# clownrat6/Tissue-Image-Segmentation

Hardware: NVIDIA B200
Metric: postproc+eval tiles/s @1000x1000 (DIST MoNuSeg config) (higher is better)
Workload: dtype u8/int32 labels, fp32 softmax, fp64 IoU

## Files before the change

tissue-image-segmentation_b200/csrc/watershed.cu:

```cuda
#include "watershed.cuh"

namespace tiseg {

#define FULL 0xffffffffu

__global__ void k_blob_init(BlobInfo b, int W) {
    int n = blockIdx.y;
    long long o = (long long)n * b.KS;
    int k = b.count[n];
    for (int i = blockIdx.x * blockDim.x + threadIdx.x; i <= k; i += gridDim.x * blockDim.x) {
        b.root[o + i] = 0; b.ymax[o + i] = -1; b.xmin[o + i] = W; b.xmax[o + i] = -1; b.area[o + i] = 0;
        if (b.lmin) { b.lmin[o + i] = 0x7fffffff; b.lmax[o + i] = 0; }
    }
}

__global__ void __launch_bounds__(TISEG_THREADS)
k_blob_roots(Geom g, const unsigned* __restrict__ bits, const int* __restrict__ rank, BlobInfo b) {
    const long long words = (long long)g.H * g.SEG;
    const long long t = (long long)blockIdx.x * blockDim.x + threadIdx.x;
    if (t >= words) return;
    const int n = blockIdx.y;
    unsigned m = bits[(long long)n * words + t];
    if (!m) return;
    const int y = (int)(t / g.SEG), seg = (int)(t - (long long)y * g.SEG);
// ... 32 lines not shown
    __syncthreads();
    for (int base = 1; base <= k; base += 256) {
        int i = base + threadIdx.x;
        int v = i <= k ? b.area[o + i] : 0;
        s[threadIdx.x] = v;
        __syncthreads();
        for (int d = 1; d < 256; d <<= 1) {
            int t = threadIdx.x >= d ? s[threadIdx.x - d] : 0;
            __syncthreads();
            s[threadIdx.x] += t;
            __syncthreads();
        }
        int incl = s[threadIdx.x];
        int c0 = carry;
        if (i <= k) b.off[o + i] = c0 + incl - v;
        __syncthreads();
        if (threadIdx.x == 255) carry = c0 + incl;
        __syncthreads();
    }
}

__global__ void __launch_bounds__(TISEG_THREADS)
k_blob_runs(Geom g, BitPlanes p, const int* __restrict__ par, const int* __restrict__ rank, BlobInfo b, int32_t* __restrict__ out) {
    const long long words = (long long)g.H * g.SEG;
    const long long t = (long long)blockIdx.x * blockDim.x + threadIdx.x;
    if (t >= words) return;
    const int n = blockIdx.y;
    const unsigned F = p.F[(long long)n * words + t];
    if (!F) return;
    const int y = (int)(t / g.SEG), seg = (int)(t - (long long)y * g.SEG);
    for (unsigned m = F & ~(F << 1); m; m &= m - 1) {
        const int a = __ffs(m) - 1;
        const unsigned rest = ~F >> a;
        const int len = rest ? __ffs(rest) - 1 : 32 - a;
        const int x = seg * 32 + a;
        const long long o = (long long)n * b.KS + blob_id_at(p, g, n, par, rank, y, x);
        const int lo = b.lmin[o], hi = b.lmax[o];
        if (lo < hi) {
            atomicMax(&b.ymax[o], y);
            atomicMin(&b.xmin[o], x);
            atomicMax(&b.xmax[o], x + len - 1);
            atomicAdd(&b.area[o], len);
        } else {
            const int lab = lo == hi ? lo : 0;
            int32_t* dst = out + (long long)n * g.P + (long long)y * g.W + x;
            for (int k = 0; k < len; ++k) dst[k] = lab;
        }
    }
}
__global__ void __launch_bounds__(TISEG_THREADS)
k_ws_seed(long long total, const int32_t* __restrict__ markers, const int* __restrict__ par, int32_t* __restrict__ out, bool vec) {
    const long long i = flat4_index();
    if (i >= total) return;
    Pack4<int> m = ld4(markers, i, total, vec), p = ld4(par, i, total, vec), o;
#pragma unroll
    for (int k = 0; k < 4; ++k) o.v[k] = p.v[k] >= 0 ? m.v[k] : 0;
    st4(out, i, total, vec, o);
}

#define WS_NOTIN 0xFFFFu
#define WS_UNLAB 0xFFFEu
#define WS_END 0xFFFFu

#define WS_MAXCLS 16
extern __shared__ __align__(16) unsigned char ws_smem[];

struct FloodWork {
    long long* items;
    long long* gen;
    long long* ovf;
    int* count;
    int* offset;
    int* fill;
    int* cursor;
    int* ngen;
    int* gcursor;
};
#define WK_INTS (4 * WS_MAXCLS + 4)

__device__ __forceinline__ long long blob_cells(const BlobInfo& b, long long ko, int bid, int W) {
    int h = b.ymax[ko + bid] - b.root[ko + bid] / W + 1, w = b.xmax[ko + bid] - b.xmin[ko + bid] + 1;
    return (long long)(w + 2) * (h + 2);
}
__device__ __forceinline__ int blob_class(long long cells, int arena, int slots) {
    if (cells > arena) return -1;
    int cls = arena / (int)cells - 1;
    return cls >= slots ? slots - 1 : cls;
}

__global__ void __launch_bounds__(TISEG_THREADS)
k_huge_clean(Geom g, BitPlanes p, const int* __restrict__ par, const int* __restrict__ rank, BlobInfo b,
             const unsigned* __restrict__ seed_bits, long long gen_cap, int32_t* __restrict__ out) {
    const long long words = (long long)g.H * g.SEG;
    const long long t = (long long)blockIdx.x * blockDim.x + threadIdx.x;
    if (t >= words) return;
    const int y = (int)(t / g.SEG), seg = (int)(t - (long long)y * g.SEG);
    FOR_TILES(true, g, n) {
        const unsigned F = p.F[(long long)n * words + t];
        const unsigned seeds = seed_bits[(long long)n * words + t];
        for (unsigned m = F & ~(F << 1); m; m &= m - 1) {
            const int a = __ffs(m) - 1;
            const unsigned rest = ~F >> a;
            const int len = rest ? __ffs(rest) - 1 : 32 - a;
            const int x = seg * 32 + a;
            const long long ko = (long long)n * b.KS;
            const int bid = blob_id_at(p, g, n, par, rank, y, x);
            if (b.lmin[ko + bid] >= b.lmax[ko + bid] || blob_cells(b, ko, bid, g.W) <= gen_cap) continue;
            int32_t* dst = out + (long long)n * g.P + (long long)y * g.W + x;
            for (int k = 0; k < len; ++k) if (!((seeds >> (a + k)) & 1u)) dst[k] = 0;
        }
    }
}

__global__ void k_flood_count(BlobInfo b, int W, FloodWork wk, int arena, int slots) {
    int n = blockIdx.y;
    long long ko = (long long)n * b.KS;
    int B = b.count[n];
    for (int bid = 1 + blockIdx.x * blockDim.x + threadIdx.x; bid <= B; bid += gridDim.x * blockDim.x) {
        if (b.lmin && b.lmin[ko + bid] >= b.lmax[ko + bid]) {
            if (b.first && b.lmax[ko + bid] > 0 && b.lmin[ko + bid] == b.lmax[ko + bid])
                atomicMin(&b.first[ko + b.lmax[ko + bid]], b.root[ko + bid]);
            continue;
        }
        int cls = blob_class(blob_cells(b, ko, bid, W), arena, slots);
        if (cls >= 0) atomicAdd(&wk.count[cls], 1);
    }
}
__global__ void k_flood_offsets(FloodWork wk) {
    if (threadIdx.x == 0) {
        int acc = 0;
        for (int k = 0; k < WS_MAXCLS; ++k) { wk.offset[k] = acc; acc += wk.count[k]; }
    }
}
__global__ void k_flood_scatter(BlobInfo b, int W, FloodWork wk, int arena, int slots, long long gen_cap, int* huge) {
    int n = blockIdx.y;
    long long ko = (long long)n * b.KS;
    int B = b.count[n];
    for (int bid = 1 + blockIdx.x * blockDim.x + threadIdx.x; bid <= B; bid += gridDim.x * blockDim.x) {
        if (b.lmin && b.lmin[ko + bid] >= b.lmax[ko + bid]) continue;
        const long long cells = blob_cells(b, ko, bid, W);
        int cls = blob_class(cells, arena, slots);
        long long item = ((long long)n << 32) | (unsigned)bid;
        if (cls >= 0) wk.items[wk.offset[cls] + atomicAdd(&wk.fill[cls], 1)] = item;
        else {
            wk.gen[atomicAdd(wk.ngen, 1)] = item;
            if (huge && cells > gen_cap && atomicExch(&huge[n], 1) == 0) huge[gridDim.y + atomicAdd(&huge[2 * gridDim.y], 1)] = n;
        }
    }
}
__global__ void __launch_bounds__(TISEG_THREADS)
k_label_clean(Geom g, const unsigned* __restrict__ keep, int32_t* __restrict__ lab) {
    const long long words = (long long)g.H * g.SEG;
    const long long wi = (long long)blockIdx.x * TISEG_WARPS_PER_BLOCK + (threadIdx.x >> 5);
    const int lane = threadIdx.x & 31;
    if (wi >= words) return;
    const int y = (int)(wi / g.SEG), seg = (int)(wi - (long long)y * g.SEG), x = seg * 32 + lane;
    FOR_TILES(true, g, n) {
        const unsigned w = keep[(long long)n * words + wi];
        if (x < g.W && !((w >> lane) & 1u)) lab[(long long)n * g.P + (long long)y * g.W + x] = 0;
    }
}
int label_clean_listed(tiseg_ctx* c, const Geom& g, const int* list, const int* count, const unsigned* keep, int32_t* lab) {
    Geom gl = listed_geom(g, list, count);
    TISEG_LAUNCH(c, k_label_clean, dim3((unsigned)(((long long)g.H * g.SEG + TISEG_WARPS_PER_BLOCK - 1) / TISEG_WARPS_PER_BLOCK), 1),
                 TISEG_THREADS, 0, gl, keep, lab);
    return TISEG_OK;
}

__device__ __forceinline__ int fdiv(int j, unsigned magic) { return (int)__umulhi((unsigned)j, magic); }

struct SeedStats { int lmn, lmx, jseed; };
struct InForest {
    static constexpr bool kMasked = false;
    const int* tp; int root;
    __device__ __forceinline__ int load(int gi) const { return tp[gi]; }
    __device__ __forceinline__ bool in(int v) const { return v == root; }
    __device__ __forceinline__ bool seed(int, unsigned, int, int ov) const { return ov != 0; }
    __device__ __forceinline__ unsigned seed_word(int, int) const { return 0u; }
};
struct InMask {
    static constexpr bool kMasked = true;
    const uint8_t* m; const int* seed_blob; const unsigned* sbits; int SEG; int bid;
    __device__ __forceinline__ int load(int gi) const { return m[gi]; }
    __device__ __forceinline__ bool in(int v) const { return v < 255; }
    __device__ __forceinline__ unsigned seed_word(int y, int x) const { return sbits[y * SEG + (x >> 5)]; }
    __device__ __forceinline__ bool seed(int gi, unsigned word, int x, int) const {
        return ((word >> (x & 31)) & 1u) && seed_blob[gi] == bid;
    }
};

template <class IT, class LT>
__device__ __forceinline__ SeedStats stage_copy(int tid, int nthr, int W, const IT* __restrict__ I, const InForest mb,
                                                const int32_t* __restrict__ o, int root,
                                                int y0, int x0, int w, int h, unsigned short* lab, LT* lvl) {
    SeedStats st; st.lmn = 0x7fffffff; st.lmx = 0; st.jseed = 0x7fffffff;
    const int wp = w + 2, cells = wp * (h + 2);
    const unsigned magic = 0xFFFFFFFFu / (unsigned)wp + 1u;
    for (int j0 = 0; j0 < cells; j0 += 8 * nthr) {
        int gi[8];
        bool in[8];
#pragma unroll
        for (int u = 0; u < 8; ++u) {
            const int j = j0 + u * nthr + tid;
            const int ly = fdiv(j, magic), lx = j - ly * wp;
            in[u] = j < cells && ly >= 1 && ly <= h && lx >= 1 && lx <= w;
            gi[u] = in[u] ? (y0 + ly - 1) * W + x0 + lx - 1 : root;
        }
        int tpv[8], ov[8];
        IT iv[8];
#pragma unroll
        for (int u = 0; u < 8; ++u) { tpv[u] = mb.load(gi[u]); iv[u] = I[gi[u]]; ov[u] = o[gi[u]]; }
#pragma unroll
        for (int u = 0; u < 8; ++u) {
            const int j = j0 + u * nthr + tid;
            if (j < cells) {
                const bool inblob = in[u] && mb.in(tpv[u]);
                const bool seed = inblob && mb.seed(gi[u], 0u, 0, ov[u]);
                lab[j] = (unsigned short)(inblob ? (seed ? (unsigned)j : WS_UNLAB) : WS_NOTIN);
                lvl[j] = (LT)iv[u];
                if (seed) { st.lmn = min(st.lmn, ov[u]); st.lmx = max(st.lmx, ov[u]); st.jseed = min(st.jseed, j); }
            }
        }
    }
    return st;
}

__device__ __forceinline__ bool fill_if_single_marker(int lane, SeedStats st, int cells, unsigned short* lab) {
#pragma unroll
    for (int d = 16; d; d >>= 1) {
// ... 118 lines not shown
        for (int u = 0; u < 8; ++u) if (dst[u] >= 0) o[dst[u]] = val[u];
    }
}

template <class MB>
__device__ __forceinline__ void flood_blob_global(int lane, int W, int H, const uint8_t* __restrict__ I,
                                                  const MB mb, int32_t* o, int* nx, int root, int y0,
                                                  int y1, int x0, int x1, int* head, int* tail, int* first = nullptr) {
    for (int i = lane; i < 256; i += 32) { head[i] = -1; tail[i] = -1; }
    __syncwarp();
    int cur = 256;
    for (int y = y0; y <= y1; ++y) {
        for (int xb = x0; xb <= x1; xb += 32) {
            int x = xb + lane;
            bool seed = false;
            int lv = 0;
            if (x <= x1) {
                int idx = y * W + x;
                if (mb.in(mb.load(idx)) && mb.seed(idx, MB::kMasked ? mb.seed_word(y, x) : 0u, x, o[idx])) { seed = true; lv = I[idx]; }
            }
            unsigned m = __ballot_sync(FULL, seed);
            while (m) {
                int src = __ffs(m) - 1;
                m &= m - 1;
                int slv = __shfl_sync(FULL, lv, src);
                if (lane == 0) {
                    int pix = y * W + xb + src;
                    if (first) atomicMin(&first[o[pix]], pix);
                    nx[pix] = -1;
                    int t = tail[slv];
                    if (t < 0) head[slv] = pix; else nx[t] = pix;
                    tail[slv] = pix;
                    if (slv < cur) cur = slv;
                }
            }
        }
    }
    if (lane == 0) {
        for (;;) {
            while (cur < 256 && head[cur] < 0) ++cur;
            if (cur >= 256) break;
            const int pix = head[cur];
            const int nxt = nx[pix];
            head[cur] = nxt;
            if (nxt < 0) tail[cur] = -1;
            const int lab_g = o[pix];
            const int y = pix / W, x = pix - y * W;
            const int nb[4] = {pix - W, pix - 1, pix + 1, pix + W};
            const bool ok[4] = {y > 0, x > 0, x + 1 < W, y + 1 < H};
            int ov[4], lv[4];
            bool pin[4];
#pragma unroll
            for (int k = 0; k < 4; ++k) {
                pin[k] = false; ov[k] = 1; lv[k] = 0;
                if (ok[k]) { pin[k] = mb.in(mb.load(nb[k])); ov[k] = o[nb[k]]; lv[k] = I[nb[k]]; }
            }
#pragma unroll
            for (int k = 0; k < 4; ++k) {
                if (pin[k] && ov[k] == 0) {
                    o[nb[k]] = lab_g;
                    if (first) atomicMin(&first[lab_g], nb[k]);
                    nx[nb[k]] = -1;
                    int t = tail[lv[k]];
                    if (t < 0) head[lv[k]] = nb[k]; else nx[t] = nb[k];
                    tail[lv[k]] = nb[k];
                    if (lv[k] < cur) cur = lv[k];
                }
            }
        }
    }
    __syncwarp();
}

#define WP_WARPS 16
#define WP_BIG_WARPS 4
#define WP_ARENA 4224
#define WP_SMALL_ARENA (WP_ARENA / 3)
#define WP_SMALL_CLS 2
#define WP_META_BYTES (256 * 2 * 2 + 128 * 4)
#define WP_GEN_CAP (WP_ARENA * WP_BIG_WARPS + WP_SMALL_ARENA * (WP_WARPS - WP_BIG_WARPS))
#define WP_SMEM_BYTES ((size_t)WP_GEN_CAP * 6 + (size_t)WP_META_BYTES * WP_WARPS)
#define WPC_NOTIN 0xFFFFu
#define WPC_UNLAB 0xFFFEu

template <class MB>
__device__ __forceinline__ SeedStats wp_stage(int tid, int nthr, int W, const uint8_t* __restrict__ I, const MB mb,
                                              const int32_t* __restrict__ o, int root, int y0, int x0, int w, int h,
                                              unsigned* cell, unsigned* cnt32) {
    SeedStats st; st.lmn = 0x7fffffff; st.lmx = 0; st.jseed = 0x7fffffff;
    const int wp = w + 2, cells = wp * (h + 2);
    const unsigned magic = 0xFFFFFFFFu / (unsigned)wp + 1u;
    for (int j0 = 0; j0 < cells; j0 += 8 * nthr) {
        int gi[8], gy[8], gx[8];
        bool in[8];
#pragma unroll
        for (int u = 0; u < 8; ++u) {
            const int j = j0 + u * nthr + tid;
            const int ly = fdiv(j, magic), lx = j - ly * wp;
            in[u] = j < cells && ly >= 1 && ly <= h && lx >= 1 && lx <= w;
            gy[u] = y0 + ly - 1; gx[u] = x0 + lx - 1;
            gi[u] = in[u] ? gy[u] * W + gx[u] : root;
        }
        int mv[8], ov[8];
        unsigned iv[8], sw[8];
#pragma unroll
        for (int u = 0; u < 8; ++u) {
            mv[u] = mb.load(gi[u]); iv[u] = I[gi[u]]; ov[u] = MB::kMasked ? 0 : o[gi[u]];
            sw[u] = (MB::kMasked && in[u]) ? mb.seed_word(gy[u], gx[u]) : 0u;
        }
#pragma unroll
        for (int u = 0; u < 8; ++u) {
            const int j = j0 + u * nthr + tid;
            if (j < cells) {
                const bool inblob = in[u] && mb.in(mv[u]);
                const bool seed = inblob && mb.seed(gi[u], sw[u], gx[u], ov[u]);
                cell[j] = ((inblob ? (seed ? (unsigned)j : WPC_UNLAB) : WPC_NOTIN) << 16) | iv[u];
                if (inblob) atomicAdd(&cnt32[iv[u] >> 1], 1u << (16 * (iv[u] & 1u)));
                if (seed) { st.lmn = min(st.lmn, ov[u]); st.lmx = max(st.lmx, ov[u]); st.jseed = min(st.jseed, j); }
            }
        }
    }
    return st;
}

__device__ __forceinline__ int wp_prepare(int lane, int cells, const unsigned* cell, unsigned short* Q, unsigned short* head,
                                          unsigned short* tail, const unsigned* cnt32) {
    int c[8], tot = 0;
#pragma unroll
    for (int k = 0; k < 4; ++k) {
        const unsigned t = cnt32[lane * 4 + k];
        c[2 * k] = (int)(t & 0xffffu); c[2 * k + 1] = (int)(t >> 16);
        tot += c[2 * k] + c[2 * k + 1];
    }
    int incl = tot;
#pragma unroll
    for (int d = 1; d < 32; d <<= 1) { const int t = __shfl_up_sync(FULL, incl, d); if (lane >= d) incl += t; }
    int off = incl - tot;
#pragma unroll
    for (int k = 0; k < 8; ++k) { head[lane * 8 + k] = (unsigned short)off; tail[lane * 8 + k] = (unsigned short)off; off += c[k]; }
    __syncwarp();
    int smin = 256;
    for (int j0 = 0; j0 < cells; j0 += 32) {
        const int j = j0 + lane;
        const unsigned cw = j < cells ? cell[j] : (WPC_NOTIN << 16);
        const bool seed = (cw >> 16) == (unsigned)j;
        if (!__ballot_sync(FULL, seed)) continue;
        const int v = (int)(cw & 0xffffu);
        const unsigned peers = __match_any_sync(FULL, seed ? v : (0x100 | lane));
        if (seed) {
            const int leader = __ffs(peers) - 1;
            const int rank = __popc(peers & ((1u << lane) - 1u));
            const int t = tail[v];
            Q[t + rank] = (unsigned short)j;
            smin = min(smin, v);
            __syncwarp(peers);
            if (lane == leader) tail[v] = (unsigned short)(t + __popc(peers));
        }
        __syncwarp();
    }
#pragma unroll
    for (int d = 16; d; d >>= 1) smin = min(smin, __shfl_xor_sync(FULL, smin, d));
    return smin;
}

__device__ __forceinline__ void wp_flood(int lane, int wp, unsigned* cell, unsigned short* Q, unsigned short* head,
                                         unsigned short* tail, int cur) {
    const int offs[4] = {-wp, -1, 1, wp};
    for (;;) {
        const int h = head[cur], t = tail[cur];
        if (h == t) {
            int nxt = -1;
            for (int base = cur + 1; base < 256 && nxt < 0; base += 32) {
                const int l = base + lane;
                const unsigned m = __ballot_sync(FULL, l < 256 && head[l] != tail[l]);
                if (m) nxt = base + __ffs(m) - 1;
            }
            if (nxt < 0) return;
            cur = nxt;
            continue;
        }
        const int B = min(t - h, 32);
        const bool act = lane < B;
        const int e = act ? (int)Q[h + lane] : 0;
        const unsigned L = act ? cell[e] >> 16 : 0u;
        unsigned ck[4];
        bool want[4];
#pragma unroll
        for (int k = 0; k < 4; ++k) {
            ck[k] = act ? cell[e + offs[k]] : (WPC_NOTIN << 16);
            want[k] = (ck[k] >> 16) == WPC_UNLAB;
        }
#pragma unroll
        for (int k = 0; k < 4; ++k)
            if (want[k]) atomicMin(&cell[e + offs[k]], ((unsigned)(lane * 4 + k) << 16) | (ck[k] & 0xffffu));
        __syncwarp();
        unsigned won = 0;
        bool desc = false;
#pragma unroll
        for (int k = 0; k < 4; ++k)
            if (want[k] && (cell[e + offs[k]] >> 16) == (unsigned)(lane * 4 + k)) {
                won |= 1u << k;
                desc |= (int)(ck[k] & 0xffffu) < cur;
            }
        const unsigned dm = __ballot_sync(FULL, desc);
        const int istar = dm ? __ffs(dm) - 1 : B - 1;
        __syncwarp();
        const bool keep = lane <= istar;
#pragma unroll
        for (int k = 0; k < 4; ++k)
            if ((won >> k) & 1u) cell[e + offs[k]] = ((keep ? L : WPC_UNLAB) << 16) | (ck[k] & 0xffffu);
        unsigned pend = keep ? won : 0u;
        int newcur = cur;
        for (;;) {
            const unsigned anyp = __ballot_sync(FULL, pend != 0u);
            if (!anyp) break;
            const int k0 = __ffs(pend) - 1;
            const int myv = pend ? (int)((k0 == 0 ? ck[0] : k0 == 1 ? ck[1] : k0 == 2 ? ck[2] : ck[3]) & 0xffffu) : 0;
            const int v = __shfl_sync(FULL, myv, __ffs(anyp) - 1);
            unsigned mine = 0;
#pragma unroll
            for (int k = 0; k < 4; ++k) if (((pend >> k) & 1u) && (int)(ck[k] & 0xffffu) == v) mine |= 1u << k;
            const unsigned b0 = __ballot_sync(FULL, mine & 1u), b1 = __ballot_sync(FULL, mine & 2u);
            const unsigned b2 = __ballot_sync(FULL, mine & 4u), b3 = __ballot_sync(FULL, mine & 8u);
            const unsigned below = (1u << lane) - 1u;
            const int pre = __popc(b0 & below) + __popc(b1 & below) + __popc(b2 & below) + __popc(b3 & below);
            const int tot = __popc(b0) + __popc(b1) + __popc(b2) + __popc(b3);
            const int tv = tail[v];
#pragma unroll
            for (int k = 0; k < 4; ++k)
                if ((mine >> k) & 1u) Q[tv + pre + __popc(mine & ((1u << k) - 1u))] = (unsigned short)(e + offs[k]);
            __syncwarp();
            if (lane == 0) tail[v] = (unsigned short)(tv + tot);
            pend &= ~mine;
            newcur = min(newcur, v);
            __syncwarp();
        }
        if (lane == 0) head[cur] = (unsigned short)(h + istar + 1);
        __syncwarp();
        cur = newcur;
    }
}

__device__ __forceinline__ void wp_writeback(int tid, int nthr, int W, int32_t* o, int y0, int x0, int w, int h, const unsigned* cell,
                                             int* first) {
    const int wp = w + 2, cells = wp * (h + 2), anchor = y0 * W + x0;
    const unsigned magic = 0xFFFFFFFFu / (unsigned)wp + 1u;
    for (int j0 = 0; j0 < cells; j0 += 8 * nthr) {
        int dst[8], src[8];
        bool store[8];
#pragma unroll
        for (int u = 0; u < 8; ++u) {
            const int j = j0 + u * nthr + tid;
            dst[u] = -1; src[u] = anchor; store[u] = false;
            if (j < cells) {
                const unsigned L = cell[j] >> 16;
                if (L < WPC_UNLAB) {
                    const int ly = fdiv(j, magic), lx = j - ly * wp, sy = fdiv((int)L, magic), sx = (int)L - sy * wp;
                    dst[u] = (y0 + ly - 1) * W + x0 + lx - 1;
                    src[u] = (y0 + sy - 1) * W + x0 + sx - 1;
                    store[u] = L != (unsigned)j;
                }
            }
        }
        int val[8];
#pragma unroll
        for (int u = 0; u < 8; ++u) val[u] = o[src[u]];
#pragma unroll
        for (int u = 0; u < 8; ++u) if (store[u]) o[dst[u]] = val[u];
        if (first) {
#pragma unroll
            for (int u = 0; u < 8; ++u) {
                const int key = dst[u] >= 0 ? val[u] : 0;
                const int left = __shfl_up_sync(FULL, key, 1);
                if (key != 0 && ((tid & 31) == 0 || left != key)) atomicMin(&first[key], dst[u]);
            }
        }
    }
}

template <bool MASKED>
__global__ void __launch_bounds__(32 * WP_WARPS, 1)
k_ws_flood_par(Geom g, const uint8_t* __restrict__ image, BlobMember bm, BlobInfo b, FloodWork wk, int* next, int* gheads,
               int32_t* out) {
    __shared__ int s_item;
    const int warp = threadIdx.x >> 5, lane = threadIdx.x & 31;
    const int W = g.W, H = g.H;
    {
        unsigned* cell = reinterpret_cast<unsigned*>(ws_smem);
        unsigned short* Q = reinterpret_cast<unsigned short*>(cell + WP_GEN_CAP);
        unsigned short* head = reinterpret_cast<unsigned short*>(ws_smem + (size_t)WP_GEN_CAP * 6);
        unsigned short* tail = head + 256;
        unsigned* cnt32 = reinterpret_cast<unsigned*>(tail + 256);
        const int ngen = wk.ngen[0];
        for (;;) {
            __syncthreads();
            if (threadIdx.x == 0) s_item = atomicAdd(wk.gcursor, 1);
            __syncthreads();
            const int k = s_item;
            if (k >= ngen) break;
            const long long item = wk.gen[k];
            const int n = (int)(item >> 32), bid = (int)(item & 0xffffffffll);
            const long long base = (long long)n * g.P, ko = (long long)n * b.KS;
            const int root = b.root[ko + bid];
            const int y0 = root / W, y1 = b.ymax[ko + bid], x0 = b.xmin[ko + bid], x1 = b.xmax[ko + bid];
            const int w = x1 - x0 + 1, h = y1 - y0 + 1;
            const long long cells = (long long)(w + 2) * (h + 2);
            const InForest inf = {bm.par + base, root};
            const InMask inm = {MASKED ? bm.mask_img + base : nullptr, MASKED ? bm.seed_blob + base : nullptr,
                                MASKED ? bm.seed_bits + (long long)n * g.H * g.SEG : nullptr, g.SEG, bid};
            if (cells > WP_GEN_CAP) {
                if (warp == 0) {
                    int* fst = b.first ? b.first + ko : nullptr;
                    if (MASKED) flood_blob_global(lane, W, H, image + base, inm, out + base, next + base, root, y0, y1, x0, x1,
                                                  gheads + (size_t)blockIdx.x * 512, gheads + (size_t)blockIdx.x * 512 + 256, fst);
                    else flood_blob_global(lane, W, H, image + base, inf, out + base, next + base, root, y0, y1, x0, x1,
                                           gheads + (size_t)blockIdx.x * 512, gheads + (size_t)blockIdx.x * 512 + 256, fst);
                }
                continue;
            }
            for (int i = threadIdx.x; i < 128; i += blockDim.x) cnt32[i] = 0u;
            __syncthreads();
            if (MASKED) wp_stage(threadIdx.x, blockDim.x, W, image + base, inm, out + base, root, y0, x0, w, h, cell, cnt32);
            else wp_stage(threadIdx.x, blockDim.x, W, image + base, inf, out + base, root, y0, x0, w, h, cell, cnt32);
            __syncthreads();
            if (warp == 0) {
                const int smin = wp_prepare(lane, (int)cells, cell, Q, head, tail, cnt32);
                if (smin < 256) wp_flood(lane, w + 2, cell, Q, head, tail, smin);
            }
            __syncthreads();
            wp_writeback(threadIdx.x, blockDim.x, W, out + base, y0, x0, w, h, cell, b.first ? b.first + ko : nullptr);
        }
        __syncthreads();
    }
    const bool big = warp < WP_BIG_WARPS;
    const int arena = big ? WP_ARENA : WP_SMALL_ARENA;
    unsigned char* wbase = ws_smem + (big ? (size_t)warp * WP_ARENA * 6
                                          : (size_t)WP_BIG_WARPS * WP_ARENA * 6 + (size_t)(warp - WP_BIG_WARPS) * WP_SMALL_ARENA * 6);
    unsigned* cell = reinterpret_cast<unsigned*>(wbase);
    unsigned short* Q = reinterpret_cast<unsigned short*>(cell + arena);
    unsigned short* head = reinterpret_cast<unsigned short*>(ws_smem + (size_t)WP_GEN_CAP * 6 + (size_t)warp * WP_META_BYTES);
    unsigned short* tail = head + 256;
    unsigned* cnt32 = reinterpret_cast<unsigned*>(tail + 256);
    for (int cls = big ? 0 : WP_SMALL_CLS; cls < WS_MAXCLS; ++cls) {
        const int cnt = wk.count[cls];
        const long long* list = wk.items + wk.offset[cls];
        for (;;) {
            int k = 0;
            if (lane == 0) k = atomicAdd(&wk.cursor[cls], 1);
            k = __shfl_sync(FULL, k, 0);
            if (k >= cnt) break;
            const long long item = list[k];
            const int n = (int)(item >> 32), bid = (int)(item & 0xffffffffll);
            const long long base = (long long)n * g.P, ko = (long long)n * b.KS;
            const int root = b.root[ko + bid];
            const int y0 = root / W, x0 = b.xmin[ko + bid];
            const int w = b.xmax[ko + bid] - x0 + 1, h = b.ymax[ko + bid] - y0 + 1;
            const int cells = (w + 2) * (h + 2);
            for (int i = lane; i < 128; i += 32) cnt32[i] = 0u;
            __syncwarp();
            bool flood = true;
            if (MASKED) {
                const InMask inm = {bm.mask_img + base, bm.seed_blob + base, bm.seed_bits + (long long)n * g.H * g.SEG, g.SEG, bid};
                wp_stage(lane, 32, W, image + base, inm, out + base, root, y0, x0, w, h, cell, cnt32);
            } else {
                const InForest inf = {bm.par + base, root};
                SeedStats st = wp_stage(lane, 32, W, image + base, inf, out + base, root, y0, x0, w, h, cell, cnt32);
#pragma unroll
                for (int d = 16; d; d >>= 1) {
                    st.lmn = min(st.lmn, __shfl_xor_sync(FULL, st.lmn, d));
                    st.lmx = max(st.lmx, __shfl_xor_sync(FULL, st.lmx, d));
                    st.jseed = min(st.jseed, __shfl_xor_sync(FULL, st.jseed, d));
                }
                __syncwarp();
                if (st.lmx != 0 && st.lmn == st.lmx) {
                    for (int j = lane; j < cells; j += 32)
                        if ((cell[j] >> 16) == WPC_UNLAB) cell[j] = ((unsigned)st.jseed << 16) | (cell[j] & 0xffffu);
                    flood = false;
                }
            }
            __syncwarp();
            if (flood) {
                const int smin = wp_prepare(lane, cells, cell, Q, head, tail, cnt32);
                if (smin < 256) wp_flood(lane, w + 2, cell, Q, head, tail, smin);
            }
            __syncwarp();
            wp_writeback(lane, 32, W, out + base, y0, x0, w, h, cell, b.first ? b.first + ko : nullptr);
            __syncwarp();
        }
    }
}

#define WR_SORT_SMALL 1024
#define WR_SORT_MAX 16384
#define WR_GEN_CAP 28160

__device__ __forceinline__ bool blob_is_huge(const BlobInfo& b, long long ko, int bid, int W) {
    return blob_cells(b, ko, bid, W) > WR_GEN_CAP || b.area[ko + bid] > WR_SORT_MAX;
}

__global__ void k_blob_prefix(const int* __restrict__ count, int N, int* prefix) {
    if (threadIdx.x == 0) {
        int acc = 0;
        for (int n = 0; n < N; ++n) { prefix[n] = acc; acc += count[n]; }
        prefix[N] = acc;
    }
}

template <bool LARGE>
__global__ void __launch_bounds__(LARGE ? 1024 : 128)
k_rank_blobs(Geom g, const double* __restrict__ image, const int* __restrict__ par, BlobInfo b, const int* __restrict__ prefix,
             unsigned short* __restrict__ level) {
    extern __shared__ __align__(16) unsigned char rk_smem[];
    constexpr int CAP = LARGE ? WR_SORT_MAX : WR_SORT_SMALL;
    double* val = reinterpret_cast<double*>(rk_smem);
    unsigned short* rnk = reinterpret_cast<unsigned short*>(val + CAP);
    __shared__ int s_cnt, s_carry;
    const int N = g.N, W = g.W, total = prefix[N];
    for (int bi = blockIdx.x; bi < total; bi += gridDim.x) {
        int n = 0;
        while (n + 1 < N && prefix[n + 1] <= bi) ++n;
        const int bid = bi - prefix[n] + 1;
        const long long ko = (long long)n * b.KS, base = (long long)n * g.P;
        const int area = b.area[ko + bid];
        if (LARGE ? (area <= WR_SORT_SMALL || blob_is_huge(b, ko, bid, W)) : (area > WR_SORT_SMALL)) continue;
        const int root = b.root[ko + bid];
        const int y0 = root / W, x0 = b.xmin[ko + bid], w = b.xmax[ko + bid] - x0 + 1, h = b.ymax[ko + bid] - y0 + 1;
        const int box = w * h;
        const unsigned magic = 0xFFFFFFFFu / (unsigned)w + 1u;
        __syncthreads();
        if (threadIdx.x == 0) s_cnt = 0;
        __syncthreads();
        for (int j = threadIdx.x; j < box; j += blockDim.x) {
            const int ly = fdiv(j, magic), lx = j - ly * w;
            const int gi = (y0 + ly) * W + x0 + lx;
            if (par[base + gi] == root) val[atomicAdd(&s_cnt, 1)] = image[base + gi];
        }
        __syncthreads();
        const int cnt = s_cnt;
        int n2 = 1;
        while (n2 < cnt) n2 <<= 1;
        for (int j = cnt + threadIdx.x; j < n2; j += blockDim.x) val[j] = INFINITY;
        __syncthreads();
        for (int k = 2; k <= n2; k <<= 1) {
            for (int d = k >> 1; d > 0; d >>= 1) {
                for (int i = threadIdx.x; i < n2; i += blockDim.x) {
                    const int ixj = i ^ d;
                    if (ixj > i) {
                        const double a = val[i], c = val[ixj];
                        const bool up = (i & k) == 0;
                        if ((a > c) == up) { val[i] = c; val[ixj] = a; }
                    }
                }
                __syncthreads();
            }
        }
        if (threadIdx.x == 0) s_carry = 0;
        __syncthreads();
        for (int c0 = 0; c0 < cnt; c0 += blockDim.x) {
            const int i = c0 + threadIdx.x;
            const int f = (i < cnt && i > 0 && val[i] != val[i - 1]) ? 1 : 0;
            int incl = f;
            const int lane = threadIdx.x & 31, wid = threadIdx.x >> 5;
#pragma unroll
            for (int dd = 1; dd < 32; dd <<= 1) { int t = __shfl_up_sync(FULL, incl, dd); if (lane >= dd) incl += t; }
            __shared__ int wtot[32];
            if (lane == 31) wtot[wid] = incl;
            __syncthreads();
            if (wid == 0) {
                int wv = lane < (int)(blockDim.x >> 5) ? wtot[lane] : 0, wi = wv;
// ... 219 lines not shown
        HeapItem* h = heap + base + b.off[ko + bid];
        int sz = 0;
        for (int y = y0; y <= y1; ++y) {
            for (int xb = x0; xb <= x1; xb += 32) {
                int x = xb + lane;
                bool seed = false;
                double v = 0.0;
                if (x <= x1) {
                    int idx = y * W + x;
                    if (tp[idx] == root && o[idx] != 0) { seed = true; v = I[idx]; }
                }
                unsigned m = __ballot_sync(FULL, seed);
                while (m) {
                    int src = __ffs(m) - 1;
                    m &= m - 1;
                    double sv = __shfl_sync(FULL, v, src);
                    if (lane == 0) { HeapItem it; it.v = sv; it.age = 0u; it.idx = y * W + xb + src; heap_push(h, sz, it); }
                }
            }
        }
        if (lane == 0) {
            unsigned age = 0;
            while (sz > 0) {
                HeapItem e = heap_pop(h, sz);
                const int pix = e.idx;
                const int lab = o[pix];
                const int y = pix / W, x = pix - y * W;
                const int nb[4] = {pix - W, pix - 1, pix + 1, pix + W};
                const bool ok[4] = {y > 0, x > 0, x + 1 < W, y + 1 < H};
                int pv[4], ov[4];
                double vv[4];
#pragma unroll
                for (int k = 0; k < 4; ++k) {
                    pv[k] = -1; ov[k] = 1; vv[k] = 0.0;
                    if (ok[k]) { pv[k] = tp[nb[k]]; ov[k] = o[nb[k]]; vv[k] = I[nb[k]]; }
                }
#pragma unroll
                for (int k = 0; k < 4; ++k) {
                    if (pv[k] >= 0 && ov[k] == 0) {
                        o[nb[k]] = lab;
                        HeapItem it; it.v = vv[k]; it.age = ++age; it.idx = nb[k];
                        heap_push(h, sz, it);
                    }
                }
            }
        }
        __syncwarp();
    }
}

int ws_seed(tiseg_ctx* c, const Geom& g, const int32_t* markers, const int* par, int32_t* out) {
    long long total = (long long)g.N * g.P;
    TISEG_LAUNCH(c, k_ws_seed, flat4_grid(total), TISEG_THREADS, 0, total, markers, par, out, aligned16(markers, par, out));
    return TISEG_OK;
}

int blobs_describe(tiseg_ctx* c, const Geom& g, const int* par, const int* rank, const unsigned* root_bits, BlobInfo& b,
                   bool want_offsets) {
    TISEG_LAUNCH(c, k_blob_init, dim3(8, g.N), 256, 0, b, g.W);
    TISEG_LAUNCH(c, k_blob_roots, dim3((unsigned)(((long long)g.H * g.SEG + TISEG_THREADS - 1) / TISEG_THREADS), g.N), TISEG_THREADS, 0,
                 g, root_bits, rank, b);
    TISEG_LAUNCH(c, k_blob_bbox, quad_grid(g), TISEG_THREADS, 0, g, par, rank, b, (g.W % 4 == 0) && aligned16(par));
    if (want_offsets) TISEG_LAUNCH(c, k_blob_offsets, g.N, 256, 0, b);
    return TISEG_OK;
}

template <bool MASKED>
static int watershed_u8_any(tiseg_ctx* c, const Geom& g, const uint8_t* image, const BlobMember& bm, const BlobInfo& b, int32_t* out) {
    const int N = g.N;
    const size_t max_blobs = (size_t)N * ((size_t)g.P / 2 + 1);
    FloodWork wk;
    wk.items = ws<long long>(c, max_blobs);
    wk.gen = ws<long long>(c, max_blobs);
    wk.ovf = nullptr;
    int* ints = ws<int>(c, WK_INTS + 2 * (size_t)N + 1);
    int* next = ws<int>(c, (size_t)N * g.P);
    int* gheads = ws<int>(c, (size_t)c->sm_count * 512);
    if (!wk.items || !wk.gen || !ints || !next || !gheads) return TISEG_ERR_CUDA;
    wk.count = ints; wk.offset = ints + WS_MAXCLS; wk.fill = ints + 2 * WS_MAXCLS; wk.cursor = ints + 3 * WS_MAXCLS;
    wk.ngen = ints + 4 * WS_MAXCLS; wk.gcursor = wk.ngen + 2;
    int* huge = ints + WK_INTS;
    TISEG_TRY(zero(c, ints, (WK_INTS + 2 * (size_t)N + 1) * sizeof(int)));
    static_assert(WP_SMEM_BYTES + 64 <= 232448, "shared memory");
    TISEG_LAUNCH(c, k_flood_count, dim3(8, g.N), 256, 0, b, g.W, wk, WP_ARENA, WS_MAXCLS);
    TISEG_LAUNCH(c, k_flood_offsets, 1, 32, 0, wk);
    TISEG_LAUNCH(c, k_flood_scatter, dim3(8, g.N), 256, 0, b, g.W, wk, WP_ARENA, WS_MAXCLS, (long long)WP_GEN_CAP, MASKED ? huge : (int*)nullptr);
    if (MASKED) {
        Geom gh = listed_geom(g, huge + N, huge + 2 * N);
        const BitPlanes mp = {const_cast<unsigned*>(bm.mask_bits), nullptr, nullptr, nullptr, nullptr};
        TISEG_LAUNCH(c, k_huge_clean, dim3((unsigned)(((long long)g.H * g.SEG + TISEG_THREADS - 1) / TISEG_THREADS), 1), TISEG_THREADS, 0,
                     gh, mp, bm.bpar, bm.brank, b, bm.seed_bits, (long long)WP_GEN_CAP, out);
    }
    static bool attr_set = false;
    if (!attr_set) {
        TISEG_CHECK(cudaFuncSetAttribute(k_ws_flood_par<MASKED>, cudaFuncAttributeMaxDynamicSharedMemorySize, (int)WP_SMEM_BYTES));
        attr_set = true;
    }
    TISEG_LAUNCH_AS(c, "k_ws_flood_par", (k_ws_flood_par<MASKED>), c->sm_count, 32 * WP_WARPS, WP_SMEM_BYTES, g, image, bm, b,
                    wk, next, gheads, out);
    return TISEG_OK;
}

int watershed_u8_dev(tiseg_ctx* c, const Geom& g, const uint8_t* image, const int* par, const int* rank,
                     const BlobInfo& b, int32_t* out) {
    (void)rank;
    BlobMember bm;
    bm.par = par; bm.mask_img = nullptr; bm.seed_blob = nullptr; bm.seed_bits = nullptr; bm.mask_bits = nullptr; bm.bpar = nullptr; bm.brank = nullptr;
    return watershed_u8_any<false>(c, g, image, bm, b, out);
}

int watershed_u8_masked_dev(tiseg_ctx* c, const Geom& g, const uint8_t* image, const BlobMember& bm, const BlobInfo& b, int32_t* out) {
    return watershed_u8_any<true>(c, g, image, bm, b, out);
}

int blobs_ccl(tiseg_ctx* c, const Geom& g, const BitPlanes& planes, int* par, int* rank, int* first, BlobInfo& b) {
    const int N = g.N, KS = g.P + 1;
    const size_t ks = (size_t)N * KS, words = (size_t)N * g.H * g.SEG;
    int* count = ws<int>(c, (size_t)N);
    b.root = ws<int>(c, ks); b.ymax = ws<int>(c, ks); b.xmin = ws<int>(c, ks); b.xmax = ws<int>(c, ks);
    b.area = ws<int>(c, ks); b.off = nullptr; b.lmin = ws<int>(c, ks); b.lmax = ws<int>(c, ks);
    b.KS = KS; b.count = count; b.first = first;
    unsigned* lbits = ws<unsigned>(c, words);
    unsigned* fbits = ws<unsigned>(c, words);
    if (!count || !b.root || !b.ymax || !b.xmin || !b.xmax || !b.area || !b.lmin || !b.lmax || !lbits || !fbits) return TISEG_ERR_CUDA;
    TISEG_TRY(bitccl_build(c, g, planes, 1, par, lbits, fbits));
    TISEG_TRY(rank_from_bits(c, g, fbits, rank, count));
    const dim3 wg((unsigned)(((long long)g.H * g.SEG + TISEG_THREADS - 1) / TISEG_THREADS), (unsigned)N);
    TISEG_LAUNCH(c, k_blob_init, dim3(8, N), 256, 0, b, g.W);
    TISEG_LAUNCH(c, k_blob_roots, wg, TISEG_THREADS, 0, g, fbits, rank, b);
    return TISEG_OK;
}

int blobs_boxes_fill(tiseg_ctx* c, const Geom& g, const BitPlanes& planes, const int* par, const int* rank, const BlobInfo& b,
                     int32_t* out) {
    const dim3 wg((unsigned)(((long long)g.H * g.SEG + TISEG_THREADS - 1) / TISEG_THREADS), (unsigned)g.N);
    TISEG_LAUNCH(c, k_blob_runs, wg, TISEG_THREADS, 0, g, planes, par, rank, b, out);
    return TISEG_OK;
}

int watershed_f64_dev(tiseg_ctx* c, const Geom& g, const double* image, const int* par, const int* rank,
                      const BlobInfo& b, int32_t* out) {
    (void)rank;
    const int N = g.N;
    HeapItem* heap = ws<HeapItem>(c, (size_t)N * g.P);
    if (!heap || !b.off) return TISEG_ERR_CUDA;
    constexpr int WARPS = 7, ARENA = 3840, SLOTS = 16;
    constexpr size_t MULTI = (size_t)WARPS * ARENA * 8, GEN = (size_t)WR_GEN_CAP * 8;
    constexpr size_t SMEM = MULTI > GEN ? MULTI : GEN;
    static_assert(SMEM + 64 <= 232448, "shared memory");
    const size_t max_blobs = (size_t)N * ((size_t)g.P / 2 + 1);
    unsigned short* level = ws<unsigned short>(c, (size_t)N * g.P);
    int* prefix = ws<int>(c, (size_t)N + 1);
    FloodWork wk;
    wk.items = ws<long long>(c, max_blobs);
    wk.gen = ws<long long>(c, max_blobs);
    wk.ovf = ws<long long>(c, max_blobs);
    int* ints = ws<int>(c, WK_INTS);
    if (!level || !prefix || !wk.items || !wk.gen || !wk.ovf || !ints) return TISEG_ERR_CUDA;
    wk.count = ints; wk.offset = ints + WS_MAXCLS; wk.fill = ints + 2 * WS_MAXCLS; wk.cursor = ints + 3 * WS_MAXCLS;
    wk.ngen = ints + 4 * WS_MAXCLS; wk.gcursor = wk.ngen + 2;
    TISEG_TRY(zero(c, ints, WK_INTS * sizeof(int)));
    static bool attr_set = false;
    constexpr size_t RK_SMALL = (size_t)WR_SORT_SMALL * 10, RK_LARGE = (size_t)WR_SORT_MAX * 10;
    if (!attr_set) {
        TISEG_CHECK(cudaFuncSetAttribute(k_rank_blobs<true>, cudaFuncAttributeMaxDynamicSharedMemorySize, (int)RK_LARGE));
        TISEG_CHECK(cudaFuncSetAttribute((k_ws_flood_ranked<WARPS, ARENA, SLOTS>), cudaFuncAttributeMaxDynamicSharedMemorySize, (int)SMEM));
// ... 58 lines not shown
```

Measured before the change: 42820.

## Stage masked watershed blobs row-wise via cp.async with relative seed labels

For the masked watershed path, blob staging now copies image rows and seed-bit words into shared memory with cp.async in row batches, replacing per-pixel scattered global loads. Seed labels are stored relative to the blob's minimum label, with a separate seed flag bit in the cell word. Blobs whose label range does not fit are routed to the global flood path. Shared-memory histogram updates are aggregated per warp with match_any, and a new writeback skips seed pixels. This adds an alignment requirement on the level image and more complex staging code.

```diff
diff --git a/tissue-image-segmentation_b200/csrc/watershed.cu b/tissue-image-segmentation_b200/csrc/watershed.cu
--- a/tissue-image-segmentation_b200/csrc/watershed.cu
+++ b/tissue-image-segmentation_b200/csrc/watershed.cu
@@ -138,6 +138,9 @@
     int h = b.ymax[ko + bid] - b.root[ko + bid] / W + 1, w = b.xmax[ko + bid] - b.xmin[ko + bid] + 1;
     return (long long)(w + 2) * (h + 2);
 }
+__device__ __forceinline__ bool blob_fits(const BlobInfo& b, long long ko, int bid, long long cells, long long cap) {
+    return cells <= cap && (!b.lmin || b.lmax[ko + bid] - b.lmin[ko + bid] < (int)WS_UNLAB);
+}
 __device__ __forceinline__ int blob_class(long long cells, int arena, int slots) {
     if (cells > arena) return -1;
     int cls = arena / (int)cells - 1;
@@ -161,7 +164,7 @@
             const int x = seg * 32 + a;
             const long long ko = (long long)n * b.KS;
             const int bid = blob_id_at(p, g, n, par, rank, y, x);
-            if (b.lmin[ko + bid] >= b.lmax[ko + bid] || blob_cells(b, ko, bid, g.W) <= gen_cap) continue;
+            if (b.lmin[ko + bid] >= b.lmax[ko + bid] || blob_fits(b, ko, bid, blob_cells(b, ko, bid, g.W), gen_cap)) continue;
             int32_t* dst = out + (long long)n * g.P + (long long)y * g.W + x;
             for (int k = 0; k < len; ++k) if (!((seeds >> (a + k)) & 1u)) dst[k] = 0;
         }
@@ -178,7 +181,8 @@
                 atomicMin(&b.first[ko + b.lmax[ko + bid]], b.root[ko + bid]);
             continue;
         }
-        int cls = blob_class(blob_cells(b, ko, bid, W), arena, slots);
+        const long long cells = blob_cells(b, ko, bid, W);
+        int cls = blob_fits(b, ko, bid, cells, arena) ? blob_class(cells, arena, slots) : -1;
         if (cls >= 0) atomicAdd(&wk.count[cls], 1);
     }
 }
@@ -195,12 +199,12 @@
     for (int bid = 1 + blockIdx.x * blockDim.x + threadIdx.x; bid <= B; bid += gridDim.x * blockDim.x) {
         if (b.lmin && b.lmin[ko + bid] >= b.lmax[ko + bid]) continue;
         const long long cells = blob_cells(b, ko, bid, W);
-        int cls = blob_class(cells, arena, slots);
+        int cls = blob_fits(b, ko, bid, cells, arena) ? blob_class(cells, arena, slots) : -1;
         long long item = ((long long)n << 32) | (unsigned)bid;
         if (cls >= 0) wk.items[wk.offset[cls] + atomicAdd(&wk.fill[cls], 1)] = item;
         else {
             wk.gen[atomicAdd(wk.ngen, 1)] = item;
-            if (huge && cells > gen_cap && atomicExch(&huge[n], 1) == 0) huge[gridDim.y + atomicAdd(&huge[2 * gridDim.y], 1)] = n;
+            if (huge && !blob_fits(b, ko, bid, cells, gen_cap) && atomicExch(&huge[n], 1) == 0) huge[gridDim.y + atomicAdd(&huge[2 * gridDim.y], 1)] = n;
         }
     }
 }
@@ -485,45 +489,116 @@
 #define WP_SMEM_BYTES ((size_t)WP_GEN_CAP * 6 + (size_t)WP_META_BYTES * WP_WARPS)
 #define WPC_NOTIN 0xFFFFu
 #define WPC_UNLAB 0xFFFEu
-
-template <class MB>
-__device__ __forceinline__ SeedStats wp_stage(int tid, int nthr, int W, const uint8_t* __restrict__ I, const MB mb,
+#define WPC_SEED 0x100u
+
+__device__ __forceinline__ SeedStats wp_stage(int tid, int nthr, int W, const uint8_t* __restrict__ I, const InForest mb,
                                               const int32_t* __restrict__ o, int root, int y0, int x0, int w, int h,
                                               unsigned* cell, unsigned* cnt32) {
     SeedStats st; st.lmn = 0x7fffffff; st.lmx = 0; st.jseed = 0x7fffffff;
     const int wp = w + 2, cells = wp * (h + 2);
     const unsigned magic = 0xFFFFFFFFu / (unsigned)wp + 1u;
     for (int j0 = 0; j0 < cells; j0 += 8 * nthr) {
-        int gi[8], gy[8], gx[8];
+        int gi[8];
         bool in[8];
 #pragma unroll
         for (int u = 0; u < 8; ++u) {
             const int j = j0 + u * nthr + tid;
             const int ly = fdiv(j, magic), lx = j - ly * wp;
             in[u] = j < cells && ly >= 1 && ly <= h && lx >= 1 && lx <= w;
-            gy[u] = y0 + ly - 1; gx[u] = x0 + lx - 1;
-            gi[u] = in[u] ? gy[u] * W + gx[u] : root;
+            gi[u] = in[u] ? (y0 + ly - 1) * W + x0 + lx - 1 : root;
         }
         int mv[8], ov[8];
-        unsigned iv[8], sw[8];
-#pragma unroll
-        for (int u = 0; u < 8; ++u) {
-            mv[u] = mb.load(gi[u]); iv[u] = I[gi[u]]; ov[u] = MB::kMasked ? 0 : o[gi[u]];
-            sw[u] = (MB::kMasked && in[u]) ? mb.seed_word(gy[u], gx[u]) : 0u;
-        }
+        unsigned iv[8];
+#pragma unroll
+        for (int u = 0; u < 8; ++u) { mv[u] = mb.load(gi[u]); iv[u] = I[gi[u]]; ov[u] = o[gi[u]]; }
 #pragma unroll
         for (int u = 0; u < 8; ++u) {
             const int j = j0 + u * nthr + tid;
             if (j < cells) {
                 const bool inblob = in[u] && mb.in(mv[u]);
-                const bool seed = inblob && mb.seed(gi[u], sw[u], gx[u], ov[u]);
-                cell[j] = ((inblob ? (seed ? (unsigned)j : WPC_UNLAB) : WPC_NOTIN) << 16) | iv[u];
+                const bool seed = inblob && mb.seed(gi[u], 0u, 0, ov[u]);
+                cell[j] = ((inblob ? (seed ? (unsigned)j : WPC_UNLAB) : WPC_NOTIN) << 16) | (seed ? WPC_SEED : 0u) | iv[u];
                 if (inblob) atomicAdd(&cnt32[iv[u] >> 1], 1u << (16 * (iv[u] & 1u)));
                 if (seed) { st.lmn = min(st.lmn, ov[u]); st.lmx = max(st.lmx, ov[u]); st.jseed = min(st.jseed, j); }
             }
         }
     }
     return st;
+}
+
+__device__ __forceinline__ void cp_async16(void* dst, const void* src, int bytes) {
+    asm volatile("cp.async.cg.shared.global [%0], [%1], 16, %2;\n" ::"r"((unsigned)__cvta_generic_to_shared(dst)), "l"(src),
+                 "r"(bytes) : "memory");
+}
+__device__ __forceinline__ void cp_async4(void* dst, const void* src) {
+    asm volatile("cp.async.ca.shared.global [%0], [%1], 4;\n" ::"r"((unsigned)__cvta_generic_to_shared(dst)), "l"(src) : "memory");
+}
+__device__ __forceinline__ void cp_async_wait_all() { asm volatile("cp.async.commit_group;\ncp.async.wait_group 0;\n" ::: "memory"); }
+__device__ __forceinline__ void group_sync(int nthr) { if (nthr == 32) __syncwarp(); else __syncthreads(); }
+
+__device__ __forceinline__ void wp_stage_rows(int tid, int nthr, int W, int SEG, const uint8_t* __restrict__ I,
+                                              const uint8_t* iend, const uint8_t* __restrict__ M,
+                                              const unsigned* __restrict__ sbits, const int* __restrict__ seed_blob,
+                                              const int32_t* __restrict__ o, int bid, int lmin, int y0, int x0, int w, int h,
+                                              unsigned* cell, unsigned char* land, int land_bytes, unsigned* cnt32) {
+    const int wp = w + 2, cells = wp * (h + 2), lane = tid & 31;
+    const unsigned magic = 0xFFFFFFFFu / (unsigned)wp + 1u;
+    const int S = (w + 30) & ~15;
+    const int q16 = S >> 4, sw0 = x0 >> 5, NW = ((x0 + w - 1) >> 5) - sw0 + 1;
+    const int R = min(h, land_bytes / (S + 4 * NW));
+    const unsigned* lw = reinterpret_cast<const unsigned*>(land + R * S);
+    for (int r0 = 0; r0 < h; r0 += R) {
+        const int nr = min(R, h - r0);
+        for (int i = tid; i < nr * q16; i += nthr) {
+            const int r = i / q16, q = i - r * q16;
+            const uint8_t* row = I + (long long)(y0 + r0 + r) * W + x0;
+            const uint8_t* a = reinterpret_cast<const uint8_t*>(reinterpret_cast<uintptr_t>(row) & ~(uintptr_t)15) + 16 * q;
+            if (a < row + w) cp_async16(land + r * S + 16 * q, a, (int)min((long long)16, (long long)(iend - a)));
+        }
+        for (int i = tid; i < nr * NW; i += nthr) {
+            const int r = i / NW;
+            cp_async4(land + R * S + 4 * i, sbits + (long long)(y0 + r0 + r) * SEG + sw0 + (i - r * NW));
+        }
+        cp_async_wait_all();
+        group_sync(nthr);
+        const int jb = r0 == 0 ? 0 : (r0 + 1) * wp, je = r0 + nr == h ? cells : (r0 + nr + 1) * wp;
+        for (int j0 = jb; j0 < je; j0 += 4 * nthr) {
+            int gi[4], v[4], mv[4], sb[4], lab[4];
+            bool in[4], sd[4];
+#pragma unroll
+            for (int u = 0; u < 4; ++u) {
+                const int j = j0 + u * nthr + tid;
+                const int ly = fdiv(j, magic), lx = j - ly * wp;
+                in[u] = j < je && ly >= 1 && ly <= h && lx >= 1 && lx <= w;
+                gi[u] = 0; v[u] = 255; sd[u] = false;
+                if (in[u]) {
+                    const int r = ly - 1 - r0, gy = y0 + ly - 1, x = x0 + lx - 1;
+                    gi[u] = gy * W + x;
+                    const int a = (int)(reinterpret_cast<uintptr_t>(I + (long long)gy * W + x0) & 15);
+                    v[u] = land[r * S + a + lx - 1];
+                    sd[u] = (lw[r * NW + (x >> 5) - sw0] >> (x & 31)) & 1u;
+                }
+            }
+#pragma unroll
+            for (int u = 0; u < 4; ++u) {
+                mv[u] = M && in[u] ? M[gi[u]] : v[u];
+                sb[u] = sd[u] ? seed_blob[gi[u]] : -1;
+                lab[u] = sd[u] ? o[gi[u]] : 0;
+            }
+#pragma unroll
+            for (int u = 0; u < 4; ++u) {
+                const int j = j0 + u * nthr + tid;
+                const bool inb = in[u] && mv[u] < 255, seed = inb && sb[u] == bid;
+                if (j < je) {
+                    const unsigned state = inb ? (seed ? (unsigned)(lab[u] - lmin) : WPC_UNLAB) : WPC_NOTIN;
+                    cell[j] = (state << 16) | (seed ? WPC_SEED : 0u) | (unsigned)v[u];
+                }
+                const unsigned peers = __match_any_sync(FULL, inb ? v[u] : 0x100 | lane);
+                if (inb && lane == __ffs(peers) - 1) atomicAdd(&cnt32[v[u] >> 1], (unsigned)__popc(peers) << (16 * (v[u] & 1)));
+            }
+        }
+        group_sync(nthr);
+    }
 }
 
 __device__ __forceinline__ int wp_prepare(int lane, int cells, const unsigned* cell, unsigned short* Q, unsigned short* head,
@@ -546,9 +621,9 @@
     for (int j0 = 0; j0 < cells; j0 += 32) {
         const int j = j0 + lane;
         const unsigned cw = j < cells ? cell[j] : (WPC_NOTIN << 16);
-        const bool seed = (cw >> 16) == (unsigned)j;
+        const bool seed = (cw & WPC_SEED) != 0u;
         if (!__ballot_sync(FULL, seed)) continue;
-        const int v = (int)(cw & 0xffffu);
+        const int v = (int)(cw & 0xffu);
         const unsigned peers = __match_any_sync(FULL, seed ? v : (0x100 | lane));
         if (seed) {
             const int leader = __ffs(peers) - 1;
@@ -681,6 +756,30 @@
     }
 }
 
+__device__ __forceinline__ void wp_writeback_rows(int tid, int nthr, int W, int32_t* o, int y0, int x0, int w, int h,
+                                                  const unsigned* cell, int lmin, int* first) {
+    const int wp = w + 2, cells = wp * (h + 2);
+    const unsigned magic = 0xFFFFFFFFu / (unsigned)wp + 1u;
+    for (int j0 = 0; j0 < cells; j0 += 8 * nthr) {
+#pragma unroll
+        for (int u = 0; u < 8; ++u) {
+            const int j = j0 + u * nthr + tid;
+            const unsigned cw = j < cells ? cell[j] : (WPC_NOTIN << 16);
+            int dst = -1, key = 0;
+            if ((cw >> 16) < WPC_UNLAB) {
+                const int ly = fdiv(j, magic), lx = j - ly * wp;
+                dst = (y0 + ly - 1) * W + x0 + lx - 1;
+                key = lmin + (int)(cw >> 16);
+                if (!(cw & WPC_SEED)) o[dst] = key;
+            }
+            if (first) {
+                const int left = __shfl_up_sync(FULL, key, 1);
+                if (key != 0 && ((tid & 31) == 0 || left != key)) atomicMin(&first[key], dst);
+            }
+        }
+    }
+}
+
 template <bool MASKED>
 __global__ void __launch_bounds__(32 * WP_WARPS, 1)
 k_ws_flood_par(Geom g, const uint8_t* __restrict__ image, BlobMember bm, BlobInfo b, FloodWork wk, int* next, int* gheads,
@@ -688,6 +787,7 @@
     __shared__ int s_item;
     const int warp = threadIdx.x >> 5, lane = threadIdx.x & 31;
     const int W = g.W, H = g.H;
+    const uint8_t* iend = image + (long long)g.N * g.P;
     {
         unsigned* cell = reinterpret_cast<unsigned*>(ws_smem);
         unsigned short* Q = reinterpret_cast<unsigned short*>(cell + WP_GEN_CAP);
@@ -711,7 +811,7 @@
             const InForest inf = {bm.par + base, root};
             const InMask inm = {MASKED ? bm.mask_img + base : nullptr, MASKED ? bm.seed_blob + base : nullptr,
                                 MASKED ? bm.seed_bits + (long long)n * g.H * g.SEG : nullptr, g.SEG, bid};
-            if (cells > WP_GEN_CAP) {
+            if (!blob_fits(b, ko, bid, cells, WP_GEN_CAP)) {
                 if (warp == 0) {
                     int* fst = b.first ? b.first + ko : nullptr;
                     if (MASKED) flood_blob_global(lane, W, H, image + base, inm, out + base, next + base, root, y0, y1, x0, x1,
@@ -723,7 +823,10 @@
             }
             for (int i = threadIdx.x; i < 128; i += blockDim.x) cnt32[i] = 0u;
             __syncthreads();
-            if (MASKED) wp_stage(threadIdx.x, blockDim.x, W, image + base, inm, out + base, root, y0, x0, w, h, cell, cnt32);
+            if (MASKED)
+                wp_stage_rows(threadIdx.x, blockDim.x, W, g.SEG, image + base, iend, bm.mask_img == image ? nullptr : bm.mask_img + base,
+                              inm.sbits, inm.seed_blob, out + base, bid, b.lmin[ko + bid], y0, x0, w, h, cell,
+                              reinterpret_cast<unsigned char*>(Q), WP_GEN_CAP * 2, cnt32);
             else wp_stage(threadIdx.x, blockDim.x, W, image + base, inf, out + base, root, y0, x0, w, h, cell, cnt32);
             __syncthreads();
             if (warp == 0) {
@@ -731,7 +834,8 @@
                 if (smin < 256) wp_flood(lane, w + 2, cell, Q, head, tail, smin);
             }
             __syncthreads();
-            wp_writeback(threadIdx.x, blockDim.x, W, out + base, y0, x0, w, h, cell, b.first ? b.first + ko : nullptr);
+            if (MASKED) wp_writeback_rows(threadIdx.x, blockDim.x, W, out + base, y0, x0, w, h, cell, b.lmin[ko + bid], b.first ? b.first + ko : nullptr);
+            else wp_writeback(threadIdx.x, blockDim.x, W, out + base, y0, x0, w, h, cell, b.first ? b.first + ko : nullptr);
         }
         __syncthreads();
     }
@@ -763,8 +867,9 @@
             __syncwarp();
             bool flood = true;
             if (MASKED) {
-                const InMask inm = {bm.mask_img + base, bm.seed_blob + base, bm.seed_bits + (long long)n * g.H * g.SEG, g.SEG, bid};
-                wp_stage(lane, 32, W, image + base, inm, out + base, root, y0, x0, w, h, cell, cnt32);
+                wp_stage_rows(lane, 32, W, g.SEG, image + base, iend, bm.mask_img == image ? nullptr : bm.mask_img + base,
+                              bm.seed_bits + (long long)n * g.H * g.SEG, bm.seed_blob + base, out + base, bid, b.lmin[ko + bid],
+                              y0, x0, w, h, cell, reinterpret_cast<unsigned char*>(Q), arena * 2, cnt32);
             } else {
                 const InForest inf = {bm.par + base, root};
                 SeedStats st = wp_stage(lane, 32, W, image + base, inf, out + base, root, y0, x0, w, h, cell, cnt32);
@@ -787,7 +892,8 @@
                 if (smin < 256) wp_flood(lane, w + 2, cell, Q, head, tail, smin);
             }
             __syncwarp();
-            wp_writeback(lane, 32, W, out + base, y0, x0, w, h, cell, b.first ? b.first + ko : nullptr);
+            if (MASKED) wp_writeback_rows(lane, 32, W, out + base, y0, x0, w, h, cell, b.lmin[ko + bid], b.first ? b.first + ko : nullptr);
+            else wp_writeback(lane, 32, W, out + base, y0, x0, w, h, cell, b.first ? b.first + ko : nullptr);
             __syncwarp();
         }
     }
@@ -1173,6 +1279,7 @@
     int* huge = ints + WK_INTS;
     TISEG_TRY(zero(c, ints, (WK_INTS + 2 * (size_t)N + 1) * sizeof(int)));
     static_assert(WP_SMEM_BYTES + 64 <= 232448, "shared memory");
+    if (MASKED && !aligned16(image)) { set_error("watershed: the level image must be 16-byte aligned"); return TISEG_ERR_ARG; }
     TISEG_LAUNCH(c, k_flood_count, dim3(8, g.N), 256, 0, b, g.W, wk, WP_ARENA, WS_MAXCLS);
     TISEG_LAUNCH(c, k_flood_offsets, 1, 32, 0, wk);
     TISEG_LAUNCH(c, k_flood_scatter, dim3(8, g.N), 256, 0, b, g.W, wk, WP_ARENA, WS_MAXCLS, (long long)WP_GEN_CAP, MASKED ? huge : (int*)nullptr);
```

Measured after the change: 42900 (median of 6 runs). About the same (+0.2%).
